# yycho0108/qpwcnet

Measured on AMD Instinct MI355X. Metric: image-pairs/sec at 256x512 fp32, higher is better.
Workload: dtype f32; 1 GPU; BASELINE configs[1]: full 6-level PWC-Net (qpwcnet build_flower) inference, batch 8 per GPU, 256x512 fp32, channels_last, d=4 cost volume + WarpV2; global_batch=8, batch_per_gpu=8, parallelism=dp1 (pairs sharded, RCCL all-gather of the 6 per-level EPE), hipgraph=True

## Files before the change

qpwcnet_amd/csrc/encoder.hip:

```cpp
#include "common.h"

namespace qpwc {

__device__ __forceinline__ float enc_mishf(float x) {
    const float e = __builtin_amdgcn_exp2f(fminf(x, 20.0f) * 1.4426950408889634f);
    const float t = e * (e + 2.0f);
    const float m = x * (t * __builtin_amdgcn_rcpf(t + 2.0f));
#if QPWC_MISH_SELECT
    return x > 20.0f ? x : m;
#else
    return m;
#endif
}

typedef float f32x4e __attribute__((ext_vector_type(4)));

__device__ __forceinline__ float2 ld2(const float* p) { return *reinterpret_cast<const float2*>(p); }
__device__ __forceinline__ float2 ld2(const __half* p) { return __half22float2(*reinterpret_cast<const __half2*>(p)); }
__device__ __forceinline__ void st4q(float* p, float4 v) { *reinterpret_cast<float4*>(p) = v; }
__device__ __forceinline__ void st4q(__half* p, float4 v) {
    __half2 lo = __floats2half2_rn(v.x, v.y), hi = __floats2half2_rn(v.z, v.w);
    uint2 u;
    u.x = *reinterpret_cast<unsigned*>(&lo);
    u.y = *reinterpret_cast<unsigned*>(&hi);
    *reinterpret_cast<uint2*>(p) = u;
}

constexpr int kEcTH = 8, kEcTW = 16;
constexpr int kEcHW = kEcTW + 2, kEcNH = (kEcTH + 2) * kEcHW;

template <int C>
__device__ __forceinline__ int ec_slot(int q, int hp) {
    return C == 16 ? (q ^ ((hp >> 2) & 3)) : (q ^ ((hp >> 1) & (C / 4 - 1)));
}

#ifndef QPWC_ENC_NT
#define QPWC_ENC_NT 1
#endif
#ifndef QPWC_ENC16_PIPE
#define QPWC_ENC16_PIPE 1
#endif
#ifndef QPWC_UPCONV16_PIPE
#define QPWC_UPCONV16_PIPE 0
#endif
#ifndef QPWC_S2_16_PIPE
#define QPWC_S2_16_PIPE 0
#endif
#ifndef QPWC_S2_PIPE
#define QPWC_S2_PIPE 0
#endif
#ifndef QPWC_UPCONV_PIPE
#define QPWC_UPCONV_PIPE 0
#endif
#ifndef QPWC_UPCONV16_NFB_MIN_WGS
#define QPWC_UPCONV16_NFB_MIN_WGS 512
#endif
#ifndef QPWC_UPCONV256_TH
#define QPWC_UPCONV256_TH 2
#endif
#ifndef QPWC_UPCONV128_TH
#define QPWC_UPCONV128_TH 4
#endif
#ifndef QPWC_UPCONV_LDS_TOTAL
#define QPWC_UPCONV_LDS_TOTAL 0
#endif
#ifndef QPWC_UPCONV64_LDS_TOTAL
#define QPWC_UPCONV64_LDS_TOTAL 82944
#endif
#ifndef QPWC_W_NEXT_ALWAYS
#define QPWC_W_NEXT_ALWAYS 1
#endif
#ifndef QPWC_W_NEXT_ALWAYS_F16
#define QPWC_W_NEXT_ALWAYS_F16 0
#endif
#if QPWC_W_NEXT_ALWAYS
#define QPWC_LOAD_W_NEXT(END) load_w(wn, kb + 1 < (END) ? kb + 1 : kb)
#else
#define QPWC_LOAD_W_NEXT(END) do { if (kb + 1 < (END)) load_w(wn, kb + 1); } while (0)
#endif
#ifndef QPWC_ENC_NARROW_EARLY
#define QPWC_ENC_NARROW_EARLY 0
#endif
#ifdef QPWC_ENC_STAMP
__device__ long long g_enc_census[4096 * 6];
#define ENC_CENSUS(i) do { if (census_on) census_p[i] = __builtin_amdgcn_s_memtime(); } while (0)
#else
#define ENC_CENSUS(i) do { } while (0)
#endif
template <int C, int NT>
__global__ __launch_bounds__(256, 4) void conv3x3_mish_kernel(const float* __restrict__ x,
                                                              const float* __restrict__ weight,
                                                              const float* __restrict__ bias,
                                                              float* __restrict__ out, int H, int W,
                                                              int pad_h, int pad_w, int tiles_x, int tiles_y,
                                                              int groups_x) {
    constexpr int NQ = C / 4;
    constexpr int NFT = C / 16;
    constexpr int NKC = C / 16;
    constexpr int NLD = (kEcNH * NQ + 255) / 256;
    constexpr int NBUF = NT > 1 ? 2 : 1;
    __shared__ __attribute__((aligned(16))) float in_s[NBUF * kEcNH * C];
    const int tid0 = threadIdx.x;
    const int wave = __builtin_amdgcn_readfirstlane(tid0 >> 6);
    const int lane = tid0 & 63, n0 = lane & 15, g0 = lane >> 4;
    const int grp = xcd_swizzle(blockIdx.x, gridDim.x);
    const int gx0 = grp % groups_x, ty = (grp / groups_x) % tiles_y, b = grp / (groups_x * tiles_y);
    const int tx0 = gx0 * NT;
    const int Y0 = ty * kEcTH;
    const float* xb = x + (int64_t)b * H * W * C;
    const int Ho = H + pad_h, Wo = W + pad_w;
    float* ob = out + (int64_t)b * Ho * Wo * C;

    auto stage_load = [&](int tid, int tx, float4 (&v)[NLD]) {
        const int X0 = tx * kEcTW;
#pragma unroll
        for (int it = 0; it < NLD; ++it) {
            const int idx = tid + 256 * it;
            const int hp = idx / NQ, q = idx - hp * NQ;
            const int hy = hp / kEcHW, hx = hp - hy * kEcHW;
            const int gy = Y0 - 1 + hy, gx = X0 - 1 + hx;
            v[it] = (idx < kEcNH * NQ && gy >= 0 && gy < H && gx >= 0 && gx < W)
                        ? *reinterpret_cast<const float4*>(xb + ((int64_t)gy * W + gx) * C + 4 * q)
                        : make_float4(0.f, 0.f, 0.f, 0.f);
        }
    };
    auto stage_write = [&](int tid, int buf, const float4 (&v)[NLD]) {
#pragma unroll
        for (int it = 0; it < NLD; ++it) {
            const int idx = tid + 256 * it;
            const int hp = idx / NQ, q = idx - hp * NQ;
            if (idx < kEcNH * NQ)
                *reinterpret_cast<float4*>(in_s + buf * (kEcNH * C) + hp * C + 4 * ec_slot<C>(q, hp)) = v[it];
        }
    };
#ifdef QPWC_ENC_STAMP
    const bool census_on = tid0 == 0 && blockIdx.x < 4096;
    long long* census_p = g_enc_census + (blockIdx.x < 4096 ? blockIdx.x : 0) * 6;
    if (census_on)
        census_p[5] = (long long)(unsigned)__builtin_amdgcn_s_getreg((4) | (0 << 6) | (31 << 11)) |
                      ((long long)(unsigned)__builtin_amdgcn_s_getreg((20) | (0 << 6) | (31 << 11)) << 32);
#endif
    ENC_CENSUS(0);
    float4 st[NLD];
    stage_load(tid0, tx0, st);
    constexpr bool EARLYB = QPWC_ENC_NARROW_EARLY && NT == 1;
    constexpr bool EARLY = EARLYB && C == 16;
    f32x4e wpre[EARLY ? 9 : 1][EARLY ? NKC : 1];
    float4 bpre[EARLYB ? NFT : 1];
    if (EARLYB) {
        if (EARLY) {
#pragma unroll
            for (int k = 0; k < 9; ++k)
#pragma unroll
                for (int kc = 0; kc < NKC; ++kc)
                    wpre[k][kc] = *reinterpret_cast<const f32x4e*>(weight + ((int64_t)k * C + n0) * C + 16 * kc + 4 * g0);
        }
#pragma unroll
        for (int ft = 0; ft < NFT; ++ft) bpre[ft] = *reinterpret_cast<const float4*>(bias + 16 * ft + 4 * g0);
        asm volatile("s_waitcnt vmcnt(0)" ::: "memory");
    }
#ifdef QPWC_ENC_STAMP
    asm volatile("s_waitcnt vmcnt(0)" ::: "memory");
#endif
    ENC_CENSUS(1);
    stage_write(tid0, 0, st);
    __syncthreads();
    ENC_CENSUS(2);

#pragma unroll 1
    for (int t = 0; t < NT; ++t) {
        const int tx = tx0 + t;
        if (tx >= tiles_x) break;
        const bool more = t + 1 < NT && tx + 1 < tiles_x;

        const int X0 = tx * kEcTW;
        const float* tile_s = in_s + (t & (NBUF - 1)) * (kEcNH * C);
        const float* wt = weight;
        int n = n0, g = g0, tid = tid0;
        if (NT > 1) asm volatile("" : "+r"(wt), "+v"(n), "+v"(g), "+v"(tid));
        if (more) stage_load(tid, tx + 1, st);
#pragma unroll
        for (int ft = 0; ft < NFT; ++ft) {
            f32x4e wld[EARLY ? 1 : 9][EARLY ? 1 : NKC];
            if (!EARLY) {
#pragma unroll
                for (int k = 0; k < 9; ++k)
#pragma unroll
                    for (int kc = 0; kc < NKC; ++kc)
                        wld[k][kc] = *reinterpret_cast<const f32x4e*>(wt + ((int64_t)k * C + 16 * ft + n) * C + 16 * kc + 4 * g);
            }
            auto wv = [&](int k, int kc) __attribute__((always_inline)) -> f32x4e& {
                if constexpr (EARLY) return wpre[k][kc];
                else return wld[k][kc];
            };
            f32x4e acc[2];
            acc[0] = f32x4e{0.f, 0.f, 0.f, 0.f};
            acc[1] = f32x4e{0.f, 0.f, 0.f, 0.f};
#pragma unroll
            for (int ky = 0; ky < 3; ++ky)
#pragma unroll
                for (int kx = 0; kx < 3; ++kx)
#pragma unroll
                    for (int kc = 0; kc < NKC; ++kc) {
                        f32x4e bv[2];
#pragma unroll
                        for (int m = 0; m < 2; ++m) {
                            const int hp = (2 * wave + m + ky) * kEcHW + n + kx;
                            const int q = 4 * kc + g;
                            const int slot = ec_slot<C>(q, hp);
                            bv[m] = *reinterpret_cast<const f32x4e*>(tile_s + hp * C + 4 * slot);
                        }
#pragma unroll
                        for (int tt = 0; tt < 4; ++tt)
#pragma unroll
                            for (int m = 0; m < 2; ++m)
                                acc[m] = __builtin_amdgcn_mfma_f32_16x16x4f32(wv(ky * 3 + kx, kc)[tt], bv[m][tt], acc[m], 0, 0, 0);
                        if (EARLY && ft + 1 < NFT) {
                            __builtin_amdgcn_sched_barrier(0);
                            wpre[ky * 3 + kx][kc] = *reinterpret_cast<const f32x4e*>(
                                wt + ((int64_t)(ky * 3 + kx) * C + 16 * (ft + 1) + n) * C + 16 * kc + 4 * g);
                            __builtin_amdgcn_sched_barrier(0);
                        }
                    }
            if (ft == NFT - 1) ENC_CENSUS(3);
            const float4 bq = EARLYB ? bpre[ft] : *reinterpret_cast<const float4*>(bias + 16 * ft + 4 * g);
#pragma unroll
            for (int m = 0; m < 2; ++m) {
                const int gy = Y0 + 2 * wave + m, gx = X0 + n;
                if (gy < H && gx < W)
                    *reinterpret_cast<float4*>(ob + ((int64_t)gy * Wo + gx) * C + 16 * ft + 4 * g) =
                        make_float4(enc_mishf(acc[m][0] + bq.x), enc_mishf(acc[m][1] + bq.y),
                                    enc_mishf(acc[m][2] + bq.z), enc_mishf(acc[m][3] + bq.w));
            }
        }
        if (pad_w > 0 && X0 + kEcTW >= W) {
            for (int i = tid; i < kEcTH * pad_w * NQ; i += 256) {
                const int q = i % NQ, r = i / NQ, col = r % pad_w, row = r / pad_w;
                const int gy = Y0 + row;
                if (gy < H) *reinterpret_cast<float4*>(ob + ((int64_t)gy * Wo + W + col) * C + 4 * q) = make_float4(0.f, 0.f, 0.f, 0.f);
            }
        }
        if (pad_h > 0 && Y0 + kEcTH >= H) {
            const int x_end = (X0 + kEcTW >= W) ? Wo : X0 + kEcTW;
            for (int i = tid; i < pad_h * (x_end - X0) * NQ; i += 256) {
                const int q = i % NQ, r = i / NQ, col = r % (x_end - X0), row = r / (x_end - X0);
                *reinterpret_cast<float4*>(ob + ((int64_t)(H + row) * Wo + X0 + col) * C + 4 * q) = make_float4(0.f, 0.f, 0.f, 0.f);
            }
        }
        ENC_CENSUS(4);
        if (more) {
            stage_write(tid, (t + 1) & (NBUF - 1), st);
            __syncthreads();
        }
    }
}

constexpr int kEwSlots = 5;
constexpr unsigned kEwOob = 0x80000000u;

template <int C, int TH>
struct EwShape {
    static constexpr int NKB = C / 32;
    static constexpr int NS = 9 * NKB;
    static constexpr int NH = (TH + 2) * kEcHW;
    static constexpr int NHI = (NH * 8 + 255) / 256;
    static constexpr int HBLK = 4 * NHI * 1024;
    static constexpr int WBASE = 2 * HBLK;
    static constexpr int LDS = WBASE + 4 * kEwSlots * 2048;
    static_assert(NKB % 2 == 0, "the K-loop walks pairs of 32-channel blocks");
};

__device__ __forceinline__ void ew_wait_vm(int n) {
    switch (n) {
#define EW_W(k) case k: asm volatile("s_waitcnt vmcnt(" #k ")" ::: "memory"); break;
        EW_W(1) EW_W(2) EW_W(3) EW_W(4) EW_W(5) EW_W(6) EW_W(7) EW_W(8) EW_W(9) EW_W(10) EW_W(11) EW_W(12)
#undef EW_W
        default: asm volatile("s_waitcnt vmcnt(0)" ::: "memory"); break;
    }
}

__device__ __forceinline__ void ew_dma16(__amdgpu_buffer_rsrc_t r, char* lds, unsigned voff, int soff) {
#ifdef __HIP_DEVICE_COMPILE__
    typedef __attribute__((address_space(3))) void* lds_ptr_t;
    __builtin_amdgcn_raw_ptr_buffer_load_lds(r, (lds_ptr_t)lds, 16, voff, soff, 0, 0);
#endif
}

__device__ __forceinline__ void ew_pin_agpr(f32x4e& v) {
#ifdef __HIP_DEVICE_COMPILE__
    asm volatile("" : "+a"(v));
#endif
}

template <int C, int TH>
__global__ __launch_bounds__(256, (2 * EwShape<C, TH>::LDS <= 160 * 1024) ? 2 : 1) void conv3x3_mish_ring_kernel(
    const float* __restrict__ x, const float* __restrict__ weight, const float* __restrict__ bias,
    float* __restrict__ out, int H, int W, int pad_h, int pad_w, int tiles_x, int tiles_y, int n_tiles) {
    using S = EwShape<C, TH>;
    __shared__ __attribute__((aligned(1024))) char smem[S::LDS];
    const int tid = threadIdx.x;
    const int wave = __builtin_amdgcn_readfirstlane(tid >> 6);
    const int lane = tid & 63, n = lane & 15, g = lane >> 4;
    const int slice = blockIdx.x / n_tiles;
    const int tile = xcd_swizzle(blockIdx.x % n_tiles, n_tiles);
    const int tx = tile % tiles_x, ty = (tile / tiles_x) % tiles_y, b = tile / (tiles_x * tiles_y);
    const int X0 = tx * kEcTW, Y0 = ty * TH;
    const int fo = 64 * slice + 16 * wave;
    const __amdgpu_buffer_rsrc_t rx = __builtin_amdgcn_make_buffer_rsrc(
        const_cast<float*>(x) + (int64_t)b * H * W * C, 0, H * W * C * 4, 0x00020000);
    const __amdgpu_buffer_rsrc_t rw = __builtin_amdgcn_make_buffer_rsrc(const_cast<float*>(weight), 0, 9 * C * C * 4, 0x00020000);

    unsigned hoff[S::NHI];
#pragma unroll
    for (int j = 0; j < S::NHI; ++j) {
        const int i = (wave * S::NHI + j) * 64 + lane;
        const int hp = i >> 3, q = (i & 7) ^ (hp & 7);
        const int hy = hp / kEcHW, hx = hp - hy * kEcHW;
        const int gy = Y0 - 1 + hy, gx = X0 - 1 + hx;
        hoff[j] = (hp < S::NH && gy >= 0 && gy < H && gx >= 0 && gx < W) ? (unsigned)(((gy * W + gx) * C + 4 * q) * 4) : kEwOob;
    }
    const unsigned woff = (unsigned)(((fo + n) * C + 4 * g) * 4);
    auto issue_h = [&](int kb) __attribute__((always_inline)) {
#pragma unroll
        for (int j = 0; j < S::NHI; ++j)
            ew_dma16(rx, smem + (kb & 1) * S::HBLK + (wave * S::NHI + j) * 1024, hoff[j], kb * 128);
    };
    auto issue_w = [&](int s) __attribute__((always_inline)) {
        const int sc = s < S::NS ? s : S::NS - 1;
        const int kb = sc / 9, tap = sc - 9 * kb;
        char* dst = smem + S::WBASE + ((s % kEwSlots) * 4 + wave) * 2048;
#pragma unroll
        for (int kc = 0; kc < 2; ++kc)
            ew_dma16(rw, dst + kc * 1024, woff, (tap * C * C + 32 * kb + 16 * kc) * 4);
    };
    f32x4e wa[2][2], pb[2][2][TH];
    auto read = [&](int s, int buf) __attribute__((always_inline)) {
        const int kb = s / 9, tap = s - 9 * kb, ky = tap / 3, kx = tap - 3 * ky;
        const char* ws = smem + S::WBASE + ((s % kEwSlots) * 4 + wave) * 2048 + lane * 16;
        const char* hs = smem + (kb & 1) * S::HBLK;
#pragma unroll
        for (int kc = 0; kc < 2; ++kc) {
            wa[buf][kc] = *reinterpret_cast<const f32x4e*>(ws + kc * 1024);
#pragma unroll
            for (int m = 0; m < TH; ++m) {
                const int hp = (m + ky) * kEcHW + n + kx;
                pb[buf][kc][m] = *reinterpret_cast<const f32x4e*>(hs + hp * 128 + 16 * ((4 * kc + g) ^ (hp & 7)));
            }
        }
    };
    f32x4e acc[TH];
#pragma unroll
    for (int m = 0; m < TH; ++m) {
        acc[m] = f32x4e{0.f, 0.f, 0.f, 0.f};
        ew_pin_agpr(acc[m]);
    }

    issue_h(0);
#pragma unroll
    for (int s = 0; s < kEwSlots - 1; ++s) issue_w(s);
    ew_wait_vm(2 * (kEwSlots - 2));
    __builtin_amdgcn_s_barrier();
    read(0, 0);

    auto pair = [&](int p, const bool LAST) __attribute__((always_inline)) {
#pragma unroll
        for (int t = 0; t < 18; ++t) {
            const int s = 18 * p + t;
            const bool more = !(LAST && t == 17);
            if (more) {
                const int tb = t % 9;
                const bool h_young = tb >= 1 && tb <= kEwSlots - 2 && !(LAST && t >= 9);
                ew_wait_vm(2 * (kEwSlots - 3) + (h_young ? S::NHI : 0));
                if (tb == 8) {
                    asm volatile("s_waitcnt lgkmcnt(0)" ::: "memory");
                    __builtin_amdgcn_s_barrier();
                }
            }
            issue_w(s + kEwSlots - 1);
            if (t == 0) issue_h(2 * p + 1);
            if (t == 9 && !LAST) issue_h(2 * p + 2);
            if (more) read(s + 1, (t + 1) & 1);
            __builtin_amdgcn_sched_barrier(0);
#pragma unroll
            for (int kc = 0; kc < 2; ++kc)
#pragma unroll
                for (int tt = 0; tt < 4; ++tt)
#pragma unroll
                    for (int m = 0; m < TH; ++m)
                        acc[m] = __builtin_amdgcn_mfma_f32_16x16x4f32(wa[t & 1][kc][tt], pb[t & 1][kc][m][tt], acc[m], 0, 0, 0);
#pragma unroll
            for (int m = 0; m < TH; ++m) ew_pin_agpr(acc[m]);
            __builtin_amdgcn_sched_barrier(0);
        }
    };
#pragma unroll 1
    for (int p = 0; p < S::NKB / 2 - 1; ++p) pair(p, false);
    pair(S::NKB / 2 - 1, true);
    asm volatile("s_waitcnt vmcnt(0)" ::: "memory");

    const int Ho = H + pad_h, Wo = W + pad_w;
    float* ob = out + (int64_t)b * Ho * Wo * C;
    const float4 bq = *reinterpret_cast<const float4*>(bias + fo + 4 * g);
#pragma unroll
    for (int m = 0; m < TH; ++m) {
        const int gy = Y0 + m, gx = X0 + n;
        if (gy < H && gx < W)
            *reinterpret_cast<float4*>(ob + ((int64_t)gy * Wo + gx) * C + fo + 4 * g) =
                make_float4(enc_mishf(acc[m][0] + bq.x), enc_mishf(acc[m][1] + bq.y),
                            enc_mishf(acc[m][2] + bq.z), enc_mishf(acc[m][3] + bq.w));
    }
    if (pad_w > 0 && X0 + kEcTW >= W) {
        for (int i = tid; i < TH * pad_w * 16; i += 256) {
            const int q = i & 15, r = i >> 4, col = r % pad_w, row = r / pad_w;
            const int gy = Y0 + row;
            if (gy < H) *reinterpret_cast<float4*>(ob + ((int64_t)gy * Wo + W + col) * C + 64 * slice + 4 * q) = make_float4(0.f, 0.f, 0.f, 0.f);
        }
    }
    if (pad_h > 0 && Y0 + TH >= H) {
        const int x_end = (X0 + kEcTW >= W) ? Wo : X0 + kEcTW;
        for (int i = tid; i < pad_h * (x_end - X0) * 16; i += 256) {
            const int q = i & 15, r = i >> 4, col = r % (x_end - X0), row = r / (x_end - X0);
            *reinterpret_cast<float4*>(ob + ((int64_t)(H + row) * Wo + X0 + col) * C + 64 * slice + 4 * q) = make_float4(0.f, 0.f, 0.f, 0.f);
        }
    }
}

template <int C, int TH>
static int conv3x3_mish_ring_launch(const void* x, const void* weight, const void* bias, void* out, int B, int H,
                                    int W, int pad_h, int pad_w, hipStream_t s) {
    const int tiles_x = (W + kEcTW - 1) / kEcTW, tiles_y = (H + TH - 1) / TH;
    const int64_t n_tiles = (int64_t)tiles_x * tiles_y * B;
    if (n_tiles * (C / 64) > INT32_MAX || (int64_t)H * W * C * 4 > INT32_MAX) {
        set_error("conv3x3_mish: too many tiles or a frame of 2 GiB or more");
        return QPWC_E_SHAPE;
    }
    hipLaunchKernelGGL((conv3x3_mish_ring_kernel<C, TH>), dim3((unsigned)(n_tiles * (C / 64))), dim3(256), 0, s,
                       (const float*)x, (const float*)weight, (const float*)bias, (float*)out, H, W, pad_h, pad_w,
                       tiles_x, tiles_y, (int)n_tiles);
    return check_launch("conv3x3_mish_ring_kernel");
}

typedef _Float16 f16x8e __attribute__((ext_vector_type(8)));
typedef _Float16 f16x4e __attribute__((ext_vector_type(4)));

template <int CP>
__device__ __forceinline__ int f16_slot(int q, int hp) {
    return CP == 32 ? (q ^ ((0 - (hp >> 2)) & 3)) : (CP == 64 ? (q ^ ((hp >> 1) & 7)) : (q ^ (hp & 15)));
}

template <int C, int TH>
__global__ __launch_bounds__(256) void conv3x3_mish_f16_kernel(const __half* __restrict__ x,
                                                              const __half* __restrict__ weight,
                                                              const float* __restrict__ bias,
                                                              __half* __restrict__ out, int H, int W, int pad_h,
                                                              int pad_w, int tiles_x, int tiles_y, int n_tiles) {
    constexpr int CP = C < 32 ? 32 : C;
    constexpr int NQ = CP / 8, NQG = C / 8;
    constexpr int HH = TH + 2, NH = HH * kEcHW;
    constexpr int NKB = CP / 32;
    constexpr int FW = C < 64 ? C : 64, NFT = FW / 16, NSL = C / FW;
    constexpr int RW = TH / 4;
    constexpr int NST = (NH * NQ + 255) / 256;
    __shared__ __attribute__((aligned(16))) __half in_s[NH * CP];
    const int tid = threadIdx.x;
    const int wave = __builtin_amdgcn_readfirstlane(tid >> 6);
    const int lane = tid & 63, n = lane & 15, g = lane >> 4;
    const int slice = blockIdx.x / n_tiles;
    const int tile = xcd_swizzle(blockIdx.x % n_tiles, n_tiles);
    const int tx = tile % tiles_x, ty = (tile / tiles_x) % tiles_y, b = tile / (tiles_x * tiles_y);
    const int X0 = tx * kEcTW, Y0 = ty * TH;
    const int f0 = FW * slice;
    const __half* xb = x + (int64_t)b * H * W * C;
    {
        uint4 st[NST];
#pragma unroll
        for (int it = 0; it < NST; ++it) {
            const int idx = tid + 256 * it;
            const int hp = idx / NQ, q = idx - hp * NQ;
            const int hy = hp / kEcHW, hx = hp - hy * kEcHW;
            const int gy = Y0 - 1 + hy, gx = X0 - 1 + hx;
            st[it] = (idx < NH * NQ && q < NQG && gy >= 0 && gy < H && gx >= 0 && gx < W)
                         ? *reinterpret_cast<const uint4*>(xb + ((int64_t)gy * W + gx) * C + 8 * q)
                         : make_uint4(0u, 0u, 0u, 0u);
        }
#pragma unroll
        for (int it = 0; it < NST; ++it) {
            const int idx = tid + 256 * it;
            const int hp = idx / NQ, q = idx - hp * NQ;
            if (idx < NH * NQ) *reinterpret_cast<uint4*>(in_s + hp * CP + 8 * f16_slot<CP>(q, hp)) = st[it];
        }
    }
    const int Ho = H + pad_h, Wo = W + pad_w;
    __half* ob = out + (int64_t)b * Ho * Wo * C;
    if (C >= 64) {
        const int fo = f0 + 16 * wave;
        f32x4e acw[TH];
#pragma unroll
        for (int r = 0; r < TH; ++r) acw[r] = f32x4e{0.f, 0.f, 0.f, 0.f};
        f16x8e wv[9], wn[9];
        auto load_w = [&](f16x8e (&w)[9], int kb) {
#pragma unroll
            for (int tap = 0; tap < 9; ++tap)
                w[tap] = *reinterpret_cast<const f16x8e*>(weight + ((int64_t)tap * C + fo + n) * C + 32 * kb + 8 * g);
        };
        load_w(wv, 0);
        __syncthreads();
        auto block = [&](f16x8e (&wv)[9], int kb) __attribute__((always_inline)) {
#if QPWC_ENC16_PIPE
            f16x8e bb[2][TH];
            auto read_b = [&](f16x8e (&bv)[TH], int tap) __attribute__((always_inline)) {
                const int ky = tap / 3, kx = tap - 3 * ky;
#pragma unroll
                for (int r = 0; r < TH; ++r) {
                    const int hp = (r + ky) * kEcHW + n + kx;
                    bv[r] = *reinterpret_cast<const f16x8e*>(in_s + hp * CP + 8 * f16_slot<CP>(4 * kb + g, hp));
                }
            };
            read_b(bb[0], 0);
#pragma unroll
            for (int tap = 0; tap < 9; ++tap) {
                if (tap + 1 < 9) read_b(bb[(tap + 1) & 1], tap + 1);
#pragma unroll
                for (int r = 0; r < TH; ++r)
                    acw[r] = __builtin_amdgcn_mfma_f32_16x16x32_f16(wv[tap], bb[tap & 1][r], acw[r], 0, 0, 0);
                __builtin_amdgcn_sched_barrier(0);
            }
#else
#pragma unroll
            for (int tap = 0; tap < 9; ++tap) {
                const int ky = tap / 3, kx = tap - 3 * ky;
#pragma unroll
                for (int r = 0; r < TH; ++r) {
                    const int hp = (r + ky) * kEcHW + n + kx;
                    const f16x8e bv = *reinterpret_cast<const f16x8e*>(in_s + hp * CP + 8 * f16_slot<CP>(4 * kb + g, hp));
                    acw[r] = __builtin_amdgcn_mfma_f32_16x16x32_f16(wv[tap], bv, acw[r], 0, 0, 0);
                }
            }
#endif
        };
#if QPWC_W_NEXT_ALWAYS_F16
        {
            int kb = 0;
#pragma unroll 1
            for (; kb + 1 < NKB; kb += 2) {
                load_w(wn, kb + 1);
                __builtin_amdgcn_sched_barrier(0);
                block(wv, kb);
                load_w(wv, kb + 2 < NKB ? kb + 2 : kb);
                __builtin_amdgcn_sched_barrier(0);
                block(wn, kb + 1);
            }
            if (kb < NKB) block(wv, kb);
        }
#else
#pragma unroll 1
        for (int kb = 0; kb < NKB; ++kb) {
            if (kb + 1 < NKB) load_w(wn, kb + 1);
            block(wv, kb);
#pragma unroll
            for (int tap = 0; tap < 9; ++tap) wv[tap] = wn[tap];
        }
#endif
        const float4 bq = *reinterpret_cast<const float4*>(bias + fo + 4 * g);
#pragma unroll
        for (int r = 0; r < TH; ++r) {
            const int gy = Y0 + r, gx = X0 + n;
            if (gy < H && gx < W) {
                f16x4e o;
                o[0] = (_Float16)enc_mishf(acw[r][0] + bq.x);
                o[1] = (_Float16)enc_mishf(acw[r][1] + bq.y);
                o[2] = (_Float16)enc_mishf(acw[r][2] + bq.z);
                o[3] = (_Float16)enc_mishf(acw[r][3] + bq.w);
                *reinterpret_cast<f16x4e*>(ob + ((int64_t)gy * Wo + gx) * C + fo + 4 * g) = o;
            }
        }
    } else {
    f32x4e acc[RW][NFT];
#pragma unroll
// ... 622 lines not shown
        for (int it = 0; it < NP; ++it) {
            const int idx = tid + 256 * it;
            const int row = idx / (kFcIW * 3), e = idx - row * (kFcIW * 3);
            const int gy = 2 * Y0 + row, gx = 2 * X0 + e / 3;
            pv[it] = make_float2(0.f, 0.f);
            if (idx < kFcIH * kFcIW * 3 && gy < H && gx < W) pv[it] = ld2(xb + ((int64_t)gy * W + 2 * X0) * 6 + 2 * e);
        }
#pragma unroll
        for (int it = 0; it < NP; ++it) {
            const int idx = tid + 256 * it;
            const int row = idx / (kFcIW * 3), e = idx - row * (kFcIW * 3);
            if (idx < kFcIH * kFcIW * 3) *reinterpret_cast<float2*>(in_s + row * (kFcIW * 6) + 2 * e) = pv[it];
        }
    }
    float wv[9];
#pragma unroll
    for (int k = 0; k < 9; ++k) wv[k] = weight[(k * 16 + n) * 4 + g];
    const float4 bq = *reinterpret_cast<const float4*>(bias + 4 * g);
    __syncthreads();

    const int f = wave >> 1;
    T* ob = out + (int64_t)(f * B + b) * Ho * Wo * 16;
    f32x4e acc[kFcTR];
#pragma unroll
    for (int r = 0; r < kFcTR; ++r) acc[r] = f32x4e{0.f, 0.f, 0.f, 0.f};
    float vb[2][kFcTR];
    auto read_tap = [&](float (&v)[kFcTR], int k) __attribute__((always_inline)) {
        const int ky = k / 3, kx = k - 3 * ky;
#pragma unroll
        for (int r = 0; r < kFcTR; ++r) {
            const int oy = kFcTR * (wave & 1) + r;
            v[r] = in_s[((2 * oy + ky) * kFcIW + 2 * n + kx) * 6 + 3 * f + (g < 3 ? g : 2)];
        }
    };
    read_tap(vb[0], 0);
#pragma unroll
    for (int k = 0; k < 9; ++k) {
        if (k + 1 < 9) read_tap(vb[(k + 1) & 1], k + 1);
        __builtin_amdgcn_sched_barrier(0);
#pragma unroll
        for (int r = 0; r < kFcTR; ++r)
            acc[r] = __builtin_amdgcn_mfma_f32_16x16x4f32(wv[k], g < 3 ? vb[k & 1][r] : 0.0f, acc[r], 0, 0, 0);
        __builtin_amdgcn_sched_barrier(0);
    }
#pragma unroll
    for (int r = 0; r < kFcTR; ++r) {
        const int gy = Y0 + kFcTR * (wave & 1) + r, gx = X0 + n;
        if (gy < Ho && gx < Wo)
            st4q(ob + ((int64_t)gy * Wo + gx) * 16 + 4 * g,
                 make_float4(enc_mishf(acc[r][0] + bq.x), enc_mishf(acc[r][1] + bq.y), enc_mishf(acc[r][2] + bq.z),
                             enc_mishf(acc[r][3] + bq.w)));
    }
}

int first_conv_mish_launch(const void* x, const void* weight, const void* bias, void* out, int B, int H, int W,
                           int layout, int dtype, hipStream_t s) {
    const int tiles_x = (W / 2 + kEcTW - 1) / kEcTW, tiles_y = (H / 2 + kFcTH - 1) / kFcTH;
    const int64_t nblk = (int64_t)tiles_x * tiles_y * B;
    if (nblk > INT32_MAX) {
        set_error("first_conv_mish: too many tiles");
        return QPWC_E_SHAPE;
    }
    if (dtype == QPWC_F32)
        hipLaunchKernelGGL(first_conv_mish_kernel<float>, dim3((unsigned)nblk), dim3(256), 0, s, (const float*)x,
                           (const float*)weight, (const float*)bias, (float*)out, B, H, W, tiles_x, tiles_y,
                           layout == QPWC_NCHW ? 1 : 0);
    else
        hipLaunchKernelGGL(first_conv_mish_kernel<__half>, dim3((unsigned)nblk), dim3(256), 0, s, (const __half*)x,
                           (const float*)weight, (const float*)bias, (__half*)out, B, H, W, tiles_x, tiles_y,
                           layout == QPWC_NCHW ? 1 : 0);
    return check_launch("first_conv_mish_kernel");
}

constexpr int kS2IH = 2 * kEcTH + 1;
constexpr int kS2PW = kEcTW + 1;

__global__ __launch_bounds__(256, 4) void conv3x3s2_mish_kernel(const float* __restrict__ x,
                                                                const float* __restrict__ weight,
                                                                const float* __restrict__ bias,
                                                                float* __restrict__ out, int H, int W,
                                                                int tiles_x, int tiles_y) {
    constexpr int CI = 16, CO = 32;
    __shared__ __attribute__((aligned(16))) float in_s[2 * kS2IH * kS2PW * CI];
    const int tid = threadIdx.x;
    const int wave = __builtin_amdgcn_readfirstlane(tid >> 6);
    const int lane = tid & 63, n = lane & 15, g = lane >> 4;
    const int tile = xcd_swizzle(blockIdx.x, gridDim.x);
    const int tx = tile % tiles_x, ty = (tile / tiles_x) % tiles_y, b = tile / (tiles_x * tiles_y);
    const int X0 = tx * kEcTW, Y0 = ty * kEcTH;
    const int Hp = H + 1, Wp = W + 1, Ho = H / 2, Wo = W / 2;
    const float* xb = x + (int64_t)b * Hp * Wp * CI;
    for (int idx = tid; idx < kS2IH * 33 * 4; idx += 256) {
        const int q = idx & 3, pxl = idx >> 2;
        const int row = pxl / 33, col = pxl - row * 33;
        const int gy = 2 * Y0 + row, gx = 2 * X0 + col;
        float4 v = make_float4(0.f, 0.f, 0.f, 0.f);
        if (gy < Hp && gx < Wp) v = *reinterpret_cast<const float4*>(xb + ((int64_t)gy * Wp + gx) * CI + 4 * q);
        const int pix = ((col & 1) * kS2IH + row) * kS2PW + (col >> 1);
        *reinterpret_cast<float4*>(in_s + pix * CI + 4 * ec_slot<CI>(q, pix)) = v;
    }
    f32x4e wv[9][2];
#pragma unroll
    for (int k = 0; k < 9; ++k)
#pragma unroll
        for (int ft = 0; ft < 2; ++ft)
            wv[k][ft] = *reinterpret_cast<const f32x4e*>(weight + ((int64_t)k * CO + 16 * ft + n) * CI + 4 * g);
    __syncthreads();

    f32x4e acc[2][2];
#pragma unroll
    for (int m = 0; m < 2; ++m)
#pragma unroll
        for (int ft = 0; ft < 2; ++ft) acc[m][ft] = f32x4e{0.f, 0.f, 0.f, 0.f};
#pragma unroll
    for (int ky = 0; ky < 3; ++ky)
#pragma unroll
        for (int kx = 0; kx < 3; ++kx) {
            f32x4e bv[2];
#pragma unroll
            for (int m = 0; m < 2; ++m) {
                const int row = 2 * (2 * wave + m) + ky;
                const int par = kx & 1, pc = n + (kx >> 1);
                const int pix = (par * kS2IH + row) * kS2PW + pc;
                bv[m] = *reinterpret_cast<const f32x4e*>(in_s + pix * CI + 4 * ec_slot<CI>(g, pix));
            }
#pragma unroll
            for (int t = 0; t < 4; ++t)
#pragma unroll
                for (int m = 0; m < 2; ++m)
#pragma unroll
                    for (int ft = 0; ft < 2; ++ft)
                        acc[m][ft] = __builtin_amdgcn_mfma_f32_16x16x4f32(wv[ky * 3 + kx][ft][t], bv[m][t], acc[m][ft], 0, 0, 0);
        }
    float* ob = out + (int64_t)b * Ho * Wo * CO;
    const float4 bq2[2] = {*reinterpret_cast<const float4*>(bias + 4 * g), *reinterpret_cast<const float4*>(bias + 16 + 4 * g)};
#pragma unroll
    for (int ft = 0; ft < 2; ++ft) {
        const float4 bq = bq2[ft];
#pragma unroll
        for (int m = 0; m < 2; ++m) {
            const int gy = Y0 + 2 * wave + m, gx = X0 + n;
            if (gy < Ho && gx < Wo)
                *reinterpret_cast<float4*>(ob + ((int64_t)gy * Wo + gx) * CO + 16 * ft + 4 * g) =
                    make_float4(enc_mishf(acc[m][ft][0] + bq.x), enc_mishf(acc[m][ft][1] + bq.y),
                                enc_mishf(acc[m][ft][2] + bq.z), enc_mishf(acc[m][ft][3] + bq.w));
        }
    }
}

template <int CI, int TH>
__global__ __launch_bounds__(256, (2 * (2 * TH + 1) * (kEcTW + 1) * CI * 4 > 80 * 1024) ? 1 : 2) void conv3x3s2_mish_wide_kernel(const float* __restrict__ x,
                                                                     const float* __restrict__ weight,
                                                                     const float* __restrict__ bias,
                                                                     float* __restrict__ out, int H, int W,
                                                                     int tiles_x, int tiles_y, int n_tiles) {
    constexpr int CO = 2 * CI, NQ = CI / 4, NKB = CI / 32;
    constexpr int IH = 2 * TH + 1, PW = kEcTW + 1;
    constexpr int NPX = IH * 33;
    constexpr int NST = (NPX * NQ + 255) / 256;
    __shared__ __attribute__((aligned(16))) float in_s[2 * IH * PW * CI];
    const int tid = threadIdx.x;
    const int wave = __builtin_amdgcn_readfirstlane(tid >> 6);
    const int lane = tid & 63, n = lane & 15, g = lane >> 4;
    const int slice = blockIdx.x / n_tiles;
    const int tile = xcd_swizzle(blockIdx.x % n_tiles, n_tiles);
    const int tx = tile % tiles_x, ty = (tile / tiles_x) % tiles_y, b = tile / (tiles_x * tiles_y);
    const int X0 = tx * kEcTW, Y0 = ty * TH;
    const int Hp = H + 1, Wp = W + 1, Ho = H / 2, Wo = W / 2;
    const int fo = 64 * slice + 16 * wave;
    const float* xb = x + (int64_t)b * Hp * Wp * CI;
    auto slot = [](int q, int pix) { return CI == 32 ? (q ^ ((pix >> 1) & 7)) : (q ^ (pix & 15)); };
    constexpr int kChunk = NST;
#pragma unroll
    for (int base = 0; base < NST; base += kChunk) {
        float4 st[kChunk];
#pragma unroll
        for (int i = 0; i < kChunk; ++i) {
            const int idx = tid + 256 * (base + i);
            const int pxl = idx / NQ, q = idx - pxl * NQ;
            const int row = pxl / 33, col = pxl - row * 33;
            const int gy = 2 * Y0 + row, gx = 2 * X0 + col;
            st[i] = (base + i < NST && idx < NPX * NQ && gy < Hp && gx < Wp)
                        ? *reinterpret_cast<const float4*>(xb + ((int64_t)gy * Wp + gx) * CI + 4 * q)
                        : make_float4(0.f, 0.f, 0.f, 0.f);
        }
#pragma unroll
        for (int i = 0; i < kChunk; ++i) {
            const int idx = tid + 256 * (base + i);
            const int pxl = idx / NQ, q = idx - pxl * NQ;
            const int row = pxl / 33, col = pxl - row * 33;
            const int pix = ((col & 1) * IH + row) * PW + (col >> 1);
            if (base + i < NST && idx < NPX * NQ) *reinterpret_cast<float4*>(in_s + pix * CI + 4 * slot(q, pix)) = st[i];
        }
    }
    f32x4e acc[TH];
#pragma unroll
    for (int m = 0; m < TH; ++m) acc[m] = f32x4e{0.f, 0.f, 0.f, 0.f};
    f32x4e wv[9][2], wn[9][2];
    auto load_w = [&](f32x4e (&w)[9][2], int kb) {
#pragma unroll
        for (int k = 0; k < 9; ++k)
#pragma unroll
            for (int kc = 0; kc < 2; ++kc)
                w[k][kc] = *reinterpret_cast<const f32x4e*>(weight + ((int64_t)k * CO + fo + n) * CI + 32 * kb + 16 * kc + 4 * g);
    };
    load_w(wv, 0);
    __syncthreads();
    auto block = [&](f32x4e (&wv)[9][2], int kb) __attribute__((always_inline)) {
#if QPWC_S2_PIPE
        f32x4e bb[2][TH];
        auto read_b = [&](f32x4e (&bv)[TH], int i) __attribute__((always_inline)) {
            const int tap = i >> 1, kc = i & 1, ky = tap / 3, kx = tap - 3 * ky;
#pragma unroll
            for (int m = 0; m < TH; ++m) {
                const int pix = ((kx & 1) * IH + 2 * m + ky) * PW + n + (kx >> 1);
                bv[m] = *reinterpret_cast<const f32x4e*>(in_s + pix * CI + 4 * slot(8 * kb + 4 * kc + g, pix));
            }
        };
        read_b(bb[0], 0);
#pragma unroll
        for (int i = 0; i < 18; ++i) {
            if (i + 1 < 18) read_b(bb[(i + 1) & 1], i + 1);
#pragma unroll
            for (int t = 0; t < 4; ++t)
#pragma unroll
                for (int m = 0; m < TH; ++m)
                    acc[m] = __builtin_amdgcn_mfma_f32_16x16x4f32(wv[i >> 1][i & 1][t], bb[i & 1][m][t], acc[m], 0, 0, 0);
            __builtin_amdgcn_sched_barrier(0);
        }
#else
#pragma unroll
        for (int ky = 0; ky < 3; ++ky)
#pragma unroll
            for (int kx = 0; kx < 3; ++kx)
#pragma unroll
                for (int kc = 0; kc < 2; ++kc) {
                    f32x4e bv[TH];
#pragma unroll
                    for (int m = 0; m < TH; ++m) {
                        const int pix = ((kx & 1) * IH + 2 * m + ky) * PW + n + (kx >> 1);
                        bv[m] = *reinterpret_cast<const f32x4e*>(in_s + pix * CI + 4 * slot(8 * kb + 4 * kc + g, pix));
                    }
#pragma unroll
                    for (int t = 0; t < 4; ++t)
#pragma unroll
                        for (int m = 0; m < TH; ++m)
                            acc[m] = __builtin_amdgcn_mfma_f32_16x16x4f32(wv[ky * 3 + kx][kc][t], bv[m][t], acc[m], 0, 0, 0);
                }
#endif
    };
#if QPWC_W_NEXT_ALWAYS
    {
        int kb = 0;
#pragma unroll 1
        for (; kb + 1 < NKB; kb += 2) {
            load_w(wn, kb + 1);
            __builtin_amdgcn_sched_barrier(0);
            block(wv, kb);
            load_w(wv, kb + 2 < NKB ? kb + 2 : kb);
            __builtin_amdgcn_sched_barrier(0);
            block(wn, kb + 1);
        }
        if (kb < NKB) block(wv, kb);
    }
#else
#pragma unroll 1
    for (int kb = 0; kb < NKB; ++kb) {
        if (kb + 1 < NKB) load_w(wn, kb + 1);
        block(wv, kb);
#pragma unroll
        for (int k = 0; k < 9; ++k)
#pragma unroll
            for (int kc = 0; kc < 2; ++kc) wv[k][kc] = wn[k][kc];
    }
#endif
    float* ob = out + (int64_t)b * Ho * Wo * CO;
    const float4 bq = *reinterpret_cast<const float4*>(bias + fo + 4 * g);
#pragma unroll
    for (int m = 0; m < TH; ++m) {
        const int gy = Y0 + m, gx = X0 + n;
        if (gy < Ho && gx < Wo)
            *reinterpret_cast<float4*>(ob + ((int64_t)gy * Wo + gx) * CO + fo + 4 * g) =
                make_float4(enc_mishf(acc[m][0] + bq.x), enc_mishf(acc[m][1] + bq.y),
                            enc_mishf(acc[m][2] + bq.z), enc_mishf(acc[m][3] + bq.w));
    }
}

template <int CI, int TH>
static int conv3x3s2_mish_wide_launch(const void* x, const void* weight, const void* bias, void* out, int B,
                                      int H, int W, hipStream_t s) {
    const int tiles_x = (W / 2 + kEcTW - 1) / kEcTW, tiles_y = (H / 2 + TH - 1) / TH;
    const int64_t n_tiles = (int64_t)tiles_x * tiles_y * B;
    const int slices = 2 * CI / 64;
    if (n_tiles * slices > INT32_MAX) {
        set_error("conv3x3s2_mish: too many tiles");
        return QPWC_E_SHAPE;
    }
    hipLaunchKernelGGL((conv3x3s2_mish_wide_kernel<CI, TH>), dim3((unsigned)(n_tiles * slices)), dim3(256), 0, s,
                       (const float*)x, (const float*)weight, (const float*)bias, (float*)out, H, W, tiles_x, tiles_y,
                       (int)n_tiles);
    return check_launch("conv3x3s2_mish_wide_kernel");
}

int conv3x3s2_mish_any_launch(const void* x, const void* weight, const void* bias, void* out, int B, int H, int W,
                              int CI, hipStream_t s);

int conv3x3s2_mish_launch(const void* x, const void* weight, const void* bias, void* out, int B, int H, int W,
                          hipStream_t s) {
    const int tiles_x = (W / 2 + kEcTW - 1) / kEcTW, tiles_y = (H / 2 + kEcTH - 1) / kEcTH;
    const int64_t nblk = (int64_t)tiles_x * tiles_y * B;
    if (nblk > INT32_MAX) {
        set_error("conv3x3s2_mish: too many tiles");
        return QPWC_E_SHAPE;
    }
    hipLaunchKernelGGL(conv3x3s2_mish_kernel, dim3((unsigned)nblk), dim3(256), 0, s, (const float*)x,
                       (const float*)weight, (const float*)bias, (float*)out, H, W, tiles_x, tiles_y);
    return check_launch("conv3x3s2_mish_kernel");
}

int conv3x3s2_mish_any_launch(const void* x, const void* weight, const void* bias, void* out, int B, int H, int W,
                              int CI, hipStream_t s) {
    switch (CI) {
        case 16: return conv3x3s2_mish_launch(x, weight, bias, out, B, H, W, s);
        case 32: return conv3x3s2_mish_wide_launch<32, 4>(x, weight, bias, out, B, H, W, s);
        case 64: return conv3x3s2_mish_wide_launch<64, 2>(x, weight, bias, out, B, H, W, s);
        case 128: return conv3x3s2_mish_wide_launch<128, 2>(x, weight, bias, out, B, H, W, s);
        default: set_error("conv3x3s2_mish: C_in=%d not in {16,32,64,128}", CI); return QPWC_E_SHAPE;
    }
}

template <int CI, int TH>
__global__ __launch_bounds__(256) void conv3x3s2_mish_f16_kernel(const __half* __restrict__ x,
                                                                const __half* __restrict__ weight,
                                                                const float* __restrict__ bias,
                                                                __half* __restrict__ out, int H, int W, int tiles_x,
                                                                int tiles_y, int n_tiles) {
    constexpr int CO = 2 * CI;
    constexpr int CP = CI < 32 ? 32 : CI;
    constexpr int NQ = CP / 8, NQG = CI / 8, NKB = CP / 32;
    constexpr int IH = 2 * TH + 1, PW = kEcTW + 1;
    constexpr int NB = CO / 16;
    constexpr int WB = NB < 4 ? NB : 4, WR = 4 / WB;
    constexpr int RW = TH / WR;
    constexpr int NCH = IH * (2 * kEcTW + 1) * NQ;
    constexpr int NST = (NCH + 255) / 256;
    __shared__ __attribute__((aligned(16))) __half in_s[2 * IH * PW * CP];
    const int tid = threadIdx.x;
    const int wave = __builtin_amdgcn_readfirstlane(tid >> 6);
    const int lane = tid & 63, n = lane & 15, g = lane >> 4;
    const int slice = blockIdx.x / n_tiles;
    const int tile = xcd_swizzle(blockIdx.x % n_tiles, n_tiles);
    const int tx = tile % tiles_x, ty = (tile / tiles_x) % tiles_y, b = tile / (tiles_x * tiles_y);
    const int X0 = tx * kEcTW, Y0 = ty * TH;
    const int Hp = H + 1, Wp = W + 1, Ho = H / 2, Wo = W / 2;
    const __half* xb = x + (int64_t)b * Hp * Wp * CI;
    {
        uint4 st[NST];
#pragma unroll
        for (int it = 0; it < NST; ++it) {
            const int idx = tid + 256 * it;
            const int q = idx % NQ, pc = idx / NQ;
            const int row = pc / (2 * kEcTW + 1), col = pc - row * (2 * kEcTW + 1);
            const int gy = 2 * Y0 + row, gx = 2 * X0 + col;
            st[it] = (idx < NCH && q < NQG && gy < Hp && gx < Wp)
                         ? *reinterpret_cast<const uint4*>(xb + ((int64_t)gy * Wp + gx) * CI + 8 * q)
                         : make_uint4(0u, 0u, 0u, 0u);
        }
#pragma unroll
        for (int it = 0; it < NST; ++it) {
            const int idx = tid + 256 * it;
            const int q = idx % NQ, pc = idx / NQ;
            const int row = pc / (2 * kEcTW + 1), col = pc - row * (2 * kEcTW + 1);
            const int hp = ((col & 1) * IH + row) * PW + (col >> 1);
            if (idx < NCH) *reinterpret_cast<uint4*>(in_s + hp * CP + 8 * f16_slot<CP>(q, hp)) = st[it];
        }
    }
    const int blk = WB == 4 ? 4 * slice + wave : (wave % WB);
    const int r0 = WB == 4 ? 0 : (wave / WB) * RW;
    const int fo = 16 * blk;
    f32x4e acc[RW];
#pragma unroll
    for (int r = 0; r < RW; ++r) acc[r] = f32x4e{0.f, 0.f, 0.f, 0.f};
    const bool kvalid = 8 * g < CI;
    f16x8e wv[9], wn[9];
    auto load_w = [&](f16x8e (&w)[9], int kb) {
#pragma unroll
        for (int tap = 0; tap < 9; ++tap) {
            w[tap] = f16x8e{0, 0, 0, 0, 0, 0, 0, 0};
            if (kvalid) w[tap] = *reinterpret_cast<const f16x8e*>(weight + ((int64_t)tap * CO + fo + n) * CI + 32 * kb + 8 * g);
        }
    };
    load_w(wv, 0);
    __syncthreads();
    auto block = [&](f16x8e (&wv)[9], int kb) __attribute__((always_inline)) {
#if QPWC_S2_16_PIPE
        f16x8e bb[3][RW];
        auto read_b = [&](f16x8e (&bv)[RW], int tap) __attribute__((always_inline)) {
            const int ky = tap / 3, kx = tap - 3 * ky;
#pragma unroll
            for (int r = 0; r < RW; ++r) {
                const int hp = ((kx & 1) * IH + 2 * (r0 + r) + ky) * PW + n + (kx >> 1);
                bv[r] = *reinterpret_cast<const f16x8e*>(in_s + hp * CP + 8 * f16_slot<CP>(4 * kb + g, hp));
            }
        };
        read_b(bb[0], 0);
        read_b(bb[1], 1);
#pragma unroll
        for (int tap = 0; tap < 9; ++tap) {
            if (tap + 2 < 9) read_b(bb[(tap + 2) % 3], tap + 2);
#pragma unroll
            for (int r = 0; r < RW; ++r) acc[r] = __builtin_amdgcn_mfma_f32_16x16x32_f16(wv[tap], bb[tap % 3][r], acc[r], 0, 0, 0);
            __builtin_amdgcn_sched_barrier(0);
        }
#else
#pragma unroll
        for (int tap = 0; tap < 9; ++tap) {
            const int ky = tap / 3, kx = tap - 3 * ky;
#pragma unroll
            for (int r = 0; r < RW; ++r) {
                const int hp = ((kx & 1) * IH + 2 * (r0 + r) + ky) * PW + n + (kx >> 1);
                const f16x8e bv = *reinterpret_cast<const f16x8e*>(in_s + hp * CP + 8 * f16_slot<CP>(4 * kb + g, hp));
                acc[r] = __builtin_amdgcn_mfma_f32_16x16x32_f16(wv[tap], bv, acc[r], 0, 0, 0);
            }
        }
#endif
    };
#if QPWC_W_NEXT_ALWAYS_F16
    {
        int kb = 0;
#pragma unroll 1
        for (; kb + 1 < NKB; kb += 2) {
            load_w(wn, kb + 1);
            __builtin_amdgcn_sched_barrier(0);
            block(wv, kb);
            load_w(wv, kb + 2 < NKB ? kb + 2 : kb);
            __builtin_amdgcn_sched_barrier(0);
            block(wn, kb + 1);
        }
        if (kb < NKB) block(wv, kb);
    }
#else
#pragma unroll 1
    for (int kb = 0; kb < NKB; ++kb) {
        if (kb + 1 < NKB) load_w(wn, kb + 1);
        block(wv, kb);
#pragma unroll
        for (int tap = 0; tap < 9; ++tap) wv[tap] = wn[tap];
    }
#endif
    __half* ob = out + (int64_t)b * Ho * Wo * CO;
    const float4 bq = *reinterpret_cast<const float4*>(bias + fo + 4 * g);
#pragma unroll
    for (int r = 0; r < RW; ++r) {
        const int gy = Y0 + r0 + r, gx = X0 + n;
        if (gy < Ho && gx < Wo)
            st4q(ob + ((int64_t)gy * Wo + gx) * CO + fo + 4 * g,
                 make_float4(enc_mishf(acc[r][0] + bq.x), enc_mishf(acc[r][1] + bq.y), enc_mishf(acc[r][2] + bq.z),
                             enc_mishf(acc[r][3] + bq.w)));
    }
}

template <int CI, int TH>
static int conv3x3s2_mish_f16_launch_t(const void* x, const void* weight, const void* bias, void* out, int B, int H,
                                       int W, hipStream_t s) {
    constexpr int NSL = (2 * CI / 16) < 4 ? 1 : (2 * CI / 16) / 4;
    const int tiles_x = (W / 2 + kEcTW - 1) / kEcTW, tiles_y = (H / 2 + TH - 1) / TH;
    const int64_t n_tiles = (int64_t)tiles_x * tiles_y * B;
    if (n_tiles * NSL > INT32_MAX) {
        set_error("conv3x3s2_mish_f16: too many tiles");
        return QPWC_E_SHAPE;
    }
    hipLaunchKernelGGL((conv3x3s2_mish_f16_kernel<CI, TH>), dim3((unsigned)(n_tiles * NSL)), dim3(256), 0, s,
                       (const __half*)x, (const __half*)weight, (const float*)bias, (__half*)out, H, W, tiles_x,
                       tiles_y, (int)n_tiles);
    return check_launch("conv3x3s2_mish_f16_kernel");
}

int conv3x3s2_mish_f16_launch(const void* x, const void* weight, const void* bias, void* out, int B, int H, int W,
                              int CI, hipStream_t s) {
    switch (CI) {
        case 16: return conv3x3s2_mish_f16_launch_t<16, 8>(x, weight, bias, out, B, H, W, s);
        case 32: return conv3x3s2_mish_f16_launch_t<32, 8>(x, weight, bias, out, B, H, W, s);
        case 64: return conv3x3s2_mish_f16_launch_t<64, 4>(x, weight, bias, out, B, H, W, s);
        case 128: return conv3x3s2_mish_f16_launch_t<128, 2>(x, weight, bias, out, B, H, W, s);
        default: set_error("conv3x3s2_mish_f16: C_in=%d not in {16,32,64,128}", CI); return QPWC_E_SHAPE;
    }
}

int conv3x3_mish_launch(const void* x, const void* weight, const void* bias, void* out, int B, int H, int W,
                        int C, int pad_h, int pad_w, hipStream_t s) {
    const int tiles_x = (W + kEcTW - 1) / kEcTW, tiles_y = (H + kEcTH - 1) / kEcTH;
    constexpr int NT = QPWC_ENC_NT;
    const int groups_x = (tiles_x + NT - 1) / NT;
    const int64_t nblk = (int64_t)groups_x * tiles_y * B;
    if (nblk > INT32_MAX) {
        set_error("conv3x3_mish: too many tiles");
        return QPWC_E_SHAPE;
    }
    const dim3 grid((unsigned)nblk);
    if (C == 16)
        hipLaunchKernelGGL((conv3x3_mish_kernel<16, NT>), grid, dim3(256), 0, s, (const float*)x, (const float*)weight,
                           (const float*)bias, (float*)out, H, W, pad_h, pad_w, tiles_x, tiles_y, groups_x);
    else if (C == 32)
        hipLaunchKernelGGL((conv3x3_mish_kernel<32, NT>), grid, dim3(256), 0, s, (const float*)x, (const float*)weight,
                           (const float*)bias, (float*)out, H, W, pad_h, pad_w, tiles_x, tiles_y, groups_x);
    else if (C == 64)
        return conv3x3_mish_ring_launch<64, 4>(x, weight, bias, out, B, H, W, pad_h, pad_w, s);
    else if (C == 128)
        return conv3x3_mish_ring_launch<128, 4>(x, weight, bias, out, B, H, W, pad_h, pad_w, s);
    else if (C == 256)
        return conv3x3_mish_ring_launch<256, 2>(x, weight, bias, out, B, H, W, pad_h, pad_w, s);
    else {
        set_error("conv3x3_mish: C=%d not in {16,32,64,128,256}", C);
        return QPWC_E_SHAPE;
    }
    return check_launch("conv3x3_mish_kernel");
}

}

#ifdef QPWC_ENC_STAMP
extern "C" int qpwc_debug_enc_census(long long* out, int n) {
    if (n > 4096 * 6) n = 4096 * 6;
    return (int)hipMemcpyFromSymbol(out, HIP_SYMBOL(qpwc::g_enc_census), n * sizeof(long long), 0, hipMemcpyDeviceToHost);
}
#endif
```

Before: 7329 pairs/s.

## Add ring-buffered weight-streaming stride-2 conv kernel for wider encoder levels

Adds a stride-2 3x3 conv+Mish MFMA kernel that streams weight taps through a multi-slot LDS ring via buffer-load-to-LDS DMA. The input halo is stored parity-split so stride-2 reads stay contiguous. LDS is capped so two workgroups fit per CU, which is meant to hide global-load latency behind MFMA work. It replaces the wide kernel for 64 and 128 input channels, and for 32 channels only when the grid is small. The deep pipeline adds vmcnt bookkeeping and register pressure.

```diff
diff --git a/qpwcnet_amd/csrc/encoder.hip b/qpwcnet_amd/csrc/encoder.hip
--- a/qpwcnet_amd/csrc/encoder.hip
+++ b/qpwcnet_amd/csrc/encoder.hip
@@ -274,6 +274,7 @@
     switch (n) {
 #define EW_W(k) case k: asm volatile("s_waitcnt vmcnt(" #k ")" ::: "memory"); break;
         EW_W(1) EW_W(2) EW_W(3) EW_W(4) EW_W(5) EW_W(6) EW_W(7) EW_W(8) EW_W(9) EW_W(10) EW_W(11) EW_W(12)
+        EW_W(13) EW_W(14) EW_W(15) EW_W(16)
 #undef EW_W
         default: asm volatile("s_waitcnt vmcnt(0)" ::: "memory"); break;
     }
@@ -1502,6 +1503,168 @@
     return check_launch("conv3x3s2_mish_wide_kernel");
 }
 
+#ifndef QPWC_S2R_WS_MAX
+#define QPWC_S2R_WS_MAX kEwSlots
+#endif
+template <int CI, int TH>
+struct Es2Shape {
+    static constexpr int NKB = CI / 32;
+    static constexpr int NB = NKB >= 2 ? 2 : 1;
+    static constexpr int NS = 9 * NKB;
+    static constexpr int IH = 2 * TH + 1, PW = kEcTW + 1;
+    static constexpr int NH = 2 * IH * PW;
+    static constexpr int NHI = (NH * 8 + 255) / 256;
+    static constexpr int HBLK = 4 * NHI * 1024;
+    static constexpr int HSLOTS = NKB >= 2 ? 2 : 1;
+    static constexpr int WBASE = HSLOTS * HBLK;
+    static constexpr int WS = (80 * 1024 - WBASE) / 8192 < QPWC_S2R_WS_MAX ? (80 * 1024 - WBASE) / 8192 : QPWC_S2R_WS_MAX;
+    static constexpr int LDS = WBASE + 4 * WS * 2048;
+    static_assert(NKB % NB == 0 && (NB == 2 || NKB == 1), "one block, or pairs of blocks");
+    static_assert(WS >= 3 && LDS <= 80 * 1024, "two workgroups per CU");
+};
+
+template <int CI, int TH>
+__global__ __launch_bounds__(256, 2) void conv3x3s2_mish_ring_kernel(
+    const float* __restrict__ x, const float* __restrict__ weight, const float* __restrict__ bias,
+    float* __restrict__ out, int H, int W, int tiles_x, int tiles_y, int n_tiles) {
+    using S = Es2Shape<CI, TH>;
+    constexpr int CO = 2 * CI, WS = S::WS;
+    __shared__ __attribute__((aligned(1024))) char smem[S::LDS];
+    const int tid = threadIdx.x;
+    const int wave = __builtin_amdgcn_readfirstlane(tid >> 6);
+    const int lane = tid & 63, n = lane & 15, g = lane >> 4;
+    const int slice = blockIdx.x / n_tiles;
+    const int tile = xcd_swizzle(blockIdx.x % n_tiles, n_tiles);
+    const int tx = tile % tiles_x, ty = (tile / tiles_x) % tiles_y, b = tile / (tiles_x * tiles_y);
+    const int X0 = tx * kEcTW, Y0 = ty * TH;
+    const int Hp = H + 1, Wp = W + 1, Ho = H / 2, Wo = W / 2;
+    const int fo = 64 * slice + 16 * wave;
+    const float4 bq = *reinterpret_cast<const float4*>(bias + fo + 4 * g);
+    __builtin_amdgcn_sched_barrier(0);
+    const __amdgpu_buffer_rsrc_t rx = __builtin_amdgcn_make_buffer_rsrc(
+        const_cast<float*>(x) + (int64_t)b * Hp * Wp * CI, 0, Hp * Wp * CI * 4, 0x00020000);
+    const __amdgpu_buffer_rsrc_t rw = __builtin_amdgcn_make_buffer_rsrc(const_cast<float*>(weight), 0, 9 * CO * CI * 4, 0x00020000);
+
+    unsigned hoff[S::NHI];
+#pragma unroll
+    for (int j = 0; j < S::NHI; ++j) {
+        const int i = (wave * S::NHI + j) * 64 + lane;
+        const int hp = i >> 3, q = (i & 7) ^ (hp & 7);
+        const int pr = hp / S::PW, pc = hp - pr * S::PW;
+        const int par = pr >= S::IH ? 1 : 0, row = pr - par * S::IH;
+        const int col = 2 * pc + par;
+        const int gy = 2 * Y0 + row, gx = 2 * X0 + col;
+        hoff[j] = (hp < S::NH && col <= 2 * kEcTW && gy < Hp && gx < Wp) ? (unsigned)(((gy * Wp + gx) * CI + 4 * q) * 4) : kEwOob;
+    }
+    const unsigned woff = (unsigned)(((fo + n) * CI + 4 * g) * 4);
+    auto issue_h = [&](int kb) __attribute__((always_inline)) {
+#pragma unroll
+        for (int j = 0; j < S::NHI; ++j)
+            ew_dma16(rx, smem + (kb & (S::HSLOTS - 1)) * S::HBLK + (wave * S::NHI + j) * 1024, hoff[j], kb * 128);
+    };
+    auto issue_w = [&](int s) __attribute__((always_inline)) {
+        const int sc = s < S::NS ? s : S::NS - 1;
+        const int kb = sc / 9, tap = sc - 9 * kb;
+        char* dst = smem + S::WBASE + ((s % WS) * 4 + wave) * 2048;
+#pragma unroll
+        for (int kc = 0; kc < 2; ++kc)
+            ew_dma16(rw, dst + kc * 1024, woff, (tap * CO * CI + 32 * kb + 16 * kc) * 4);
+    };
+    f32x4e wa[2][2], pb[2][2][TH];
+    auto read = [&](int s, int buf) __attribute__((always_inline)) {
+        const int kb = s / 9, tap = s - 9 * kb, ky = tap / 3, kx = tap - 3 * ky;
+        const char* ws = smem + S::WBASE + ((s % WS) * 4 + wave) * 2048 + lane * 16;
+        const char* hs = smem + (kb & (S::HSLOTS - 1)) * S::HBLK;
+#pragma unroll
+        for (int kc = 0; kc < 2; ++kc) {
+            wa[buf][kc] = *reinterpret_cast<const f32x4e*>(ws + kc * 1024);
+#pragma unroll
+            for (int m = 0; m < TH; ++m) {
+                const int hp = ((kx & 1) * S::IH + 2 * m + ky) * S::PW + n + (kx >> 1);
+                pb[buf][kc][m] = *reinterpret_cast<const f32x4e*>(hs + hp * 128 + 16 * ((4 * kc + g) ^ (hp & 7)));
+            }
+        }
+    };
+    f32x4e acc[TH];
+#pragma unroll
+    for (int m = 0; m < TH; ++m) {
+        acc[m] = f32x4e{0.f, 0.f, 0.f, 0.f};
+        ew_pin_agpr(acc[m]);
+    }
+
+    issue_h(0);
+#pragma unroll
+    for (int s = 0; s < WS - 1; ++s) issue_w(s);
+    ew_wait_vm(2 * (WS - 2));
+    __builtin_amdgcn_s_barrier();
+    read(0, 0);
+
+    constexpr int NT = 9 * S::NB;
+    auto trip = [&](int p, const bool LAST) __attribute__((always_inline)) {
+#pragma unroll
+        for (int t = 0; t < NT; ++t) {
+            const int s = NT * p + t, j = t / 9, tb = t - 9 * j;
+            const bool more = !(LAST && t == NT - 1);
+            const bool h_req = !(LAST && j == S::NB - 1);
+            if (more) {
+                const bool h_young = h_req && tb >= 1 && tb <= WS - 2;
+                ew_wait_vm(2 * (WS - 3) + (h_young ? S::NHI : 0));
+                if (tb == 8) {
+                    asm volatile("s_waitcnt lgkmcnt(0)" ::: "memory");
+                    __builtin_amdgcn_s_barrier();
+                }
+            }
+            issue_w(s + WS - 1);
+            if (tb == 0 && h_req) issue_h(S::NB * p + j + 1);
+            if (more) read(s + 1, (t + 1) & 1);
+            __builtin_amdgcn_sched_barrier(0);
+#pragma unroll
+            for (int kc = 0; kc < 2; ++kc)
+#pragma unroll
+                for (int tt = 0; tt < 4; ++tt)
+#pragma unroll
+                    for (int m = 0; m < TH; ++m)
+                        acc[m] = __builtin_amdgcn_mfma_f32_16x16x4f32(wa[t & 1][kc][tt], pb[t & 1][kc][m][tt], acc[m], 0, 0, 0);
+#pragma unroll
+            for (int m = 0; m < TH; ++m) ew_pin_agpr(acc[m]);
+            __builtin_amdgcn_sched_barrier(0);
+        }
+    };
+#pragma unroll
+    for (int p = 0; p < S::NKB / S::NB - 1; ++p) trip(p, false);
+    trip(S::NKB / S::NB - 1, true);
+    asm volatile("s_waitcnt vmcnt(0)" ::: "memory");
+
+    float* ob = out + (int64_t)b * Ho * Wo * CO;
+#pragma unroll
+    for (int m = 0; m < TH; ++m) {
+        const int gy = Y0 + m, gx = X0 + n;
+        if (gy < Ho && gx < Wo)
+            *reinterpret_cast<float4*>(ob + ((int64_t)gy * Wo + gx) * CO + fo + 4 * g) =
+                make_float4(enc_mishf(acc[m][0] + bq.x), enc_mishf(acc[m][1] + bq.y),
+                            enc_mishf(acc[m][2] + bq.z), enc_mishf(acc[m][3] + bq.w));
+    }
+}
+
+template <int CI, int TH>
+static int conv3x3s2_mish_ring_launch(const void* x, const void* weight, const void* bias, void* out, int B,
+                                      int H, int W, hipStream_t s) {
+    const int tiles_x = (W / 2 + kEcTW - 1) / kEcTW, tiles_y = (H / 2 + TH - 1) / TH;
+    const int64_t n_tiles = (int64_t)tiles_x * tiles_y * B;
+    const int slices = 2 * CI / 64;
+    if (n_tiles * slices > INT32_MAX || (int64_t)(H + 1) * (W + 1) * CI * 4 > INT32_MAX) {
+        set_error("conv3x3s2_mish: too many tiles or a frame of 2 GiB or more");
+        return QPWC_E_SHAPE;
+    }
+    hipLaunchKernelGGL((conv3x3s2_mish_ring_kernel<CI, TH>), dim3((unsigned)(n_tiles * slices)), dim3(256), 0, s,
+                       (const float*)x, (const float*)weight, (const float*)bias, (float*)out, H, W, tiles_x, tiles_y,
+                       (int)n_tiles);
+    return check_launch("conv3x3s2_mish_ring_kernel");
+}
+
+#ifndef QPWC_S2_RING32_MAX_WGS
+#define QPWC_S2_RING32_MAX_WGS 512
+#endif
 int conv3x3s2_mish_any_launch(const void* x, const void* weight, const void* bias, void* out, int B, int H, int W,
                               int CI, hipStream_t s);
 
@@ -1522,9 +1685,13 @@
                               int CI, hipStream_t s) {
     switch (CI) {
         case 16: return conv3x3s2_mish_launch(x, weight, bias, out, B, H, W, s);
-        case 32: return conv3x3s2_mish_wide_launch<32, 4>(x, weight, bias, out, B, H, W, s);
-        case 64: return conv3x3s2_mish_wide_launch<64, 2>(x, weight, bias, out, B, H, W, s);
-        case 128: return conv3x3s2_mish_wide_launch<128, 2>(x, weight, bias, out, B, H, W, s);
+        case 32: {
+            const int64_t wgs = (int64_t)((W / 2 + kEcTW - 1) / kEcTW) * ((H / 2 + 3) / 4) * B;
+            return wgs <= QPWC_S2_RING32_MAX_WGS ? conv3x3s2_mish_ring_launch<32, 4>(x, weight, bias, out, B, H, W, s)
+                                                 : conv3x3s2_mish_wide_launch<32, 4>(x, weight, bias, out, B, H, W, s);
+        }
+        case 64: return conv3x3s2_mish_ring_launch<64, 2>(x, weight, bias, out, B, H, W, s);
+        case 128: return conv3x3s2_mish_ring_launch<128, 2>(x, weight, bias, out, B, H, W, s);
         default: set_error("conv3x3s2_mish: C_in=%d not in {16,32,64,128}", CI); return QPWC_E_SHAPE;
     }
 }
```

Result: no change. 7399 pairs/s, median of 6 (+1.0%).
